# ppt0011/distributed_training

Hardware: AMD Instinct MI355X
Metric: images/sec (node) ResNet-50 at 1/2/4/8 MI355X; grad-sync bus GB/s (higher is better)
Workload: dtype bf16

## Files before the change

distributed_training_amd/_lib.py:

```python
from __future__ import annotations

import ctypes
import os
import threading

import torch

LIB_PATH = os.environ.get(
    "GSYNC_LIB", os.path.join(os.path.dirname(os.path.abspath(__file__)), "lib", "libgsync.so")
)

GS_OK = 0
GS_EINVAL, GS_EHIP, GS_ERCCL, GS_ESTATE, GS_ENOMEM, GS_ENODEV = -1, -2, -3, -4, -5, -6
GS_F32, GS_BF16, GS_F16, GS_F64, GS_I64, GS_I32, GS_U8 = 0, 1, 2, 3, 4, 5, 6
GS_DEV_HOST, GS_DEV_HIP = 0, 1
GS_SUM, GS_PROD, GS_MAX, GS_MIN, GS_AVG = 0, 1, 2, 3, 4
GS_SCALE_NONE, GS_SCALE_MUL, GS_SCALE_DIV = 0, 1, 2
GS_PLAN_SLOTS = 5
GS_RED_GROUPS = 64
GS_RED_PARTIALS = 1024
GS_BKT_AUTO_COLLECTIVE = 1
GS_BKT_GRAD_VIEW = 2
GS_BKT_NO_SCALE = 4
GS_BKT_REDUCE_SCATTER = 8
# ... 74 lines not shown
    "gs_rng_draw_u32": (_c_int, [_vp, _c_i64, _c_i64, _vp]),
    "gs_randperm": (_c_int, [ctypes.c_uint64, _c_i64, _vp]),
    "gs_distributed_sampler_indices": (_c_int, [_c_i64, _c_int, _c_int, _c_int, ctypes.c_uint64, _c_i64, _c_int,
                                                _vp, _c_i64, _p_i64]),
    "gs_crop_flip_params": (_c_int, [_vp, _c_i64, _c_int, _c_int, _c_int, _c_int, _c_int, _c_int, _vp, _c_i64,
                                     _vp]),
    "gs_image_augment": (_c_int, [_c_int, _c_int, _vp, _vp, _c_i64, _c_int, _c_int, _c_int, _c_int, _c_int, _c_int,
                                  _vp, _c_i64, _vp, _c_int, _c_int, _vp, _vp]),
    "gs_image_augment_mix": (_c_int, [_c_int, _c_int, _vp, _vp, _c_i64, _c_int, _c_int, _c_int, _c_int, _c_int, _c_int,
                                      _vp, _vp, _c_i64, _vp, _c_int, _c_int, _vp, _vp, _vp, _vp]),
    "gs_bn_bwd_partials": (_c_int, [_c_i64, _c_int]),
    "gs_bn_bwd_reduce": (_c_int, [_vp, _vp, _vp, _vp, _vp, _vp, _c_i64, _c_i64, _c_int, _vp]),
    "gs_bn_bwd_reduce_fork": (_c_int, [_vp, _vp, _vp, _vp, _vp, _vp, _vp, _c_i64, _c_i64, _c_int, _vp]),
    "gs_bn_bwd_dx": (_c_int, [_vp, _vp, _vp, _vp, _vp, _vp, _vp, _c_i64, _vp, _vp, _vp, _c_i64, _c_int, _vp]),
    "gs_add_relu_fwd": (_c_int, [_vp, _vp, _c_i64, _vp]),
    "gs_relu_maxpool_fwd": (_c_int, [_vp, _vp, _vp, _c_i64, _c_int, _c_int, _c_int, _vp]),
    "gs_maxpool_bwd": (_c_int, [_vp, _vp, _vp, _vp, _c_i64, _c_int, _c_int, _c_int, _vp]),
    "gs_relu_mask_fwd": (_c_int, [_vp, _vp, _c_i64, _vp]),
    "gs_add_relu_mask_fwd": (_c_int, [_vp, _vp, _vp, _c_i64, _vp]),
    "gs_relu_maxpool_mask_fwd": (_c_int, [_vp, _vp, _vp, _vp, _c_i64, _c_int, _c_int, _c_int, _vp]),
    "gs_bn_bwd_reduce_bits": (_c_int, [_vp, _vp, _vp, _vp, _vp, _vp, _c_i64, _c_i64, _c_int, _vp]),
    "gs_bn_bwd_reduce_fork_bits": (_c_int, [_vp, _vp, _vp, _vp, _vp, _vp, _vp, _c_i64, _c_i64, _c_int, _vp]),
    "gs_bn_bwd_dx_bits": (_c_int, [_vp, _vp, _vp, _vp, _vp, _vp, _vp, _c_i64, _vp, _vp, _vp, _c_i64, _c_int, _vp]),
    "gs_bn_infer_act": (_c_int, [_vp, _vp, _vp, _vp, _vp, _vp, _c_d, _c_int, _vp, _c_i64, _c_int, _vp]),
    "gs_bn_infer_relu_maxpool": (_c_int, [_vp, _vp, _vp, _vp, _vp, _c_d, _vp, _c_i64, _c_int, _c_int, _c_int, _vp]),
    "gs_eval_accumulate": (_c_int, [_c_int, _vp, _c_int, _vp, _c_i64, _c_i64, _c_i64, _c_i64, _p_i32, _c_int, _c_i64,
                                    _vp, _vp, _vp]),
    "gs_xent_fwd": (_c_int, [_c_int, _vp, _c_int, _vp, _c_i64, _c_i64, _c_i64, _c_i64, _c_f, _vp, _vp, _p_i32, _c_int,
                             _vp, _vp]),
    "gs_xent_bwd": (_c_int, [_c_int, _vp, _c_int, _vp, _c_i64, _c_i64, _c_i64, _c_i64, _c_f, _c_int, _vp, _vp, _vp, _vp,
                             _c_i64, _vp]),
    "gs_xent_mix_fwd": (_c_int, [_c_int, _vp, _c_int, _vp, _vp, _vp, _c_i64, _c_i64, _c_i64, _c_i64, _c_f, _vp, _vp,
                                 _p_i32, _c_int, _vp, _vp]),
    "gs_xent_mix_bwd": (_c_int, [_c_int, _vp, _c_int, _vp, _vp, _vp, _c_i64, _c_i64, _c_i64, _c_i64, _c_f, _c_int, _vp,
                                 _vp, _vp, _vp, _c_i64, _vp]),
    "gs_clip_coef":(_c_int, [_c_int, _vp, _c_f, _c_f, _vp, _vp, _vp]),
    "gs_unscale_check": (_c_int, [_vp, _c_int, _c_int, _vp, _vp, _vp]),
    "gs_sgd_step": (
        _c_int,
        [_vp, _c_int, _c_int, _c_d, _c_d, _c_d, _c_d, _c_int, _c_int, _c_int, _vp, _vp, _vp],
    ),
    "gs_adam_step": (
        _c_int,
        [_vp, _c_int, _c_int, _c_d, _c_d, _c_d, _c_d, _c_d, _c_int, _c_int, _c_d, _c_d, _vp, _vp, _vp],
    ),
    "gs_plan_set_adapt": (_c_int, [_vp, _p_i32]),
# ... 186 lines not shown
```

distributed_training_amd/csrc/gs_bn_kernels.hip:

```cpp
#include <hip/hip_runtime.h>

#include <algorithm>
#include <climits>
#include <cmath>

#include "gs_common.h"

#ifndef GS_BN_NT
#define GS_BN_NT 0
#endif
#ifndef GS_BN_DX_RNE
#define GS_BN_DX_RNE 0
#endif

namespace gs {
namespace {

#define HIP_RET(expr)                                                               \
  do {                                                                              \
    hipError_t _e = (expr);                                                         \
    if (_e != hipSuccess)                                                           \
      return fail(GS_EHIP, std::string(#expr " failed: ") + hipGetErrorString(_e)); \
  } while (0)

// ... 103 lines not shown
#pragma unroll
  for (int i = 0; i < 8; ++i) g[i] = yf[i] <= 0.f ? 0.f : g[i];
}

enum : int { kMaskNone = 0, kMaskY = 1, kMaskBits = 2 };

__device__ __forceinline__ void relu_mask_bits(float (&g)[8], uint32_t mb) {
#pragma unroll
  for (int i = 0; i < 8; ++i) g[i] = (mb >> i) & 1u ? g[i] : 0.f;
}

__device__ __forceinline__ uint8_t mask_byte(const float (&f)[8]) {
  uint32_t mb = 0;
#pragma unroll
  for (int j = 0; j < 8; ++j) mb |= (f[j] <= 0.f ? 0u : 1u) << j;
  return static_cast<uint8_t>(mb);
}

__device__ __forceinline__ void fork_sum(float (&g)[8], const bu4& bv) {
  float b[8];
  unpack8(bv, b);
#pragma unroll
  for (int i = 0; i < 8; ++i) g[i] = __uint_as_float(to_bf16(g[i] + b[i]) << 16);
}

template <int BLOCK, int MASK, bool WRITE_G, bool FORK>
__global__ void __launch_bounds__(BLOCK, (BLOCK == kBlock && MASK == kMaskBits && !WRITE_G) ? 5 : 1)
bn_bwd_reduce_kernel(const uint16_t* __restrict__ x, const uint16_t* __restrict__ dy, const uint16_t* __restrict__ dy2,
                     const uint16_t* __restrict__ y, const uint8_t* __restrict__ mask, uint16_t* __restrict__ gout,
                     const float* __restrict__ mean, float* __restrict__ ws, int64_t R, int C, int tx_log2,
                     int64_t rpb) {
  constexpr int U = FORK ? kBnForkUnroll : kBnUnroll;
  __shared__ float s_red[BLOCK * 16];
  __shared__ double s_grp[BLOCK];
  const int t = threadIdx.x;
  const int tx = 1 << tx_log2, ty = BLOCK >> tx_log2;
  const int tx_i = t & (tx - 1), ty_i = t >> tx_log2;
  const int v = blockIdx.x * tx + tx_i;
  const bool active = v < (C >> 3);
  const int c0 = v * 8;
  const int64_t r0 = static_cast<int64_t>(blockIdx.y) * rpb;
  const int64_t r1 = std::min<int64_t>(R, r0 + rpb);

  float sg[8], sq[8], m[8];
#pragma unroll
  for (int i = 0; i < 8; ++i) {
// ... 24 lines not shown
      uint32_t mb[U] = {};
#pragma unroll
      for (int k = 0; k < U; ++k) {
        xv[k] = ld16<false>(x + off + k * step);
        dv[k] = ld16<GS_BN_NT && WRITE_G>(dy + off + k * step);
        if constexpr (FORK) bv[k] = ld16<GS_BN_NT>(dy2 + off + k * step);
        if constexpr (MASK == kMaskY) yv[k] = ld16<GS_BN_NT && WRITE_G>(y + off + k * step);
        if constexpr (MASK == kMaskBits) mb[k] = mask[(off + k * step) >> 3];
      }
      if constexpr (MASK == kMaskBits) __builtin_amdgcn_sched_barrier(0);
#pragma unroll
      for (int k = 0; k < U; ++k) body(xv[k], dv[k], bv[k], yv[k], mb[k], off + k * step);
    }
    for (; r < r1; r += ty, off += step) {
      bu4 bv = {0u, 0u, 0u, 0u}, yv = {0u, 0u, 0u, 0u};
      uint32_t mb = 0;
      const bu4 xv = ld16<false>(x + off), dv = ld16<false>(dy + off);
      if constexpr (FORK) bv = ld16<false>(dy2 + off);
      if constexpr (MASK == kMaskY) yv = ld16<false>(y + off);
      if constexpr (MASK == kMaskBits) mb = mask[off >> 3];
      body(xv, dv, bv, yv, mb, off);
    }
  }
  const int F = 16 << tx_log2;
#pragma unroll
  for (int i = 0; i < 8; ++i) {
    s_red[t * 16 + 2 * i] = sg[i];
    s_red[t * 16 + 2 * i + 1] = sq[i];
  }
  __syncthreads();
  {
    const int o = t & (F - 1), grp = t >> (tx_log2 + 4);
    double a = 0.0;
#pragma unroll
    for (int k = 0; k < 16; ++k) a += static_cast<double>(s_red[(grp * 16 + k) * F + o]);
    s_grp[t] = a;
  }
  __syncthreads();
  if (t < F) {
    const int G = BLOCK / F;
    double a = 0.0;
    for (int k = 0; k < G; ++k) a += s_grp[k * F + t];
    const int ch = blockIdx.x * (tx * 8) + (t >> 1);
    if (ch < C) ws[(static_cast<int64_t>(blockIdx.y) * C + ch) * 2 + (t & 1)] = static_cast<float>(a);
  }
}

template <int BLOCK, int MASK>
__global__ void __launch_bounds__(BLOCK)
bn_bwd_dx_kernel(const uint16_t* __restrict__ x, const uint16_t* __restrict__ dy, const uint16_t* __restrict__ y,
                 const uint8_t* __restrict__ mask, const float* __restrict__ mean, const float* __restrict__ invstd, const float* __restrict__ weight,
                 const float* __restrict__ ws, int P, uint16_t* __restrict__ dx, float* __restrict__ gw,
                 float* __restrict__ gb, int64_t R, int C, int tx_log2, int64_t rpb, double inv_R) {
  __shared__ double s_fold[BLOCK * 4];
  __shared__ double s_sum[BLOCK / 2];
  const int t = threadIdx.x;
  const int tx = 1 << tx_log2, ty = BLOCK >> tx_log2;
  const int tx_i = t & (tx - 1), ty_i = t >> tx_log2;
  const int tile_c0 = blockIdx.x * (tx * 8);
  {
    const int F4 = 4 << tx_log2, G4 = BLOCK / F4;
    const int q = t & (F4 - 1), grp = t >> (tx_log2 + 2);
    double a[4] = {0.0, 0.0, 0.0, 0.0};
    if (tile_c0 + 2 * q < C) {
      const bf4* base = reinterpret_cast<const bf4*>(ws + static_cast<int64_t>(tile_c0) * 2) + q;
      const int64_t stride = C >> 1;
#pragma unroll 8
      for (int p = grp; p < P; p += G4) {
        const bf4 w4 = base[p * stride];
#pragma unroll
        for (int j = 0; j < 4; ++j) a[j] += static_cast<double>(w4[j]);
      }
    }
#pragma unroll
    for (int j = 0; j < 4; ++j) s_fold[t * 4 + j] = a[j];
    __syncthreads();
    if (t < 4 * F4) {
      double b = 0.0;
      for (int k = 0; k < G4; ++k) b += s_fold[k * 4 * F4 + t];
      s_sum[t] = b;
    }
    __syncthreads();
  }
  if (blockIdx.y == 0 && t < tx * 8 && tile_c0 + t < C) {
    gb[tile_c0 + t] = static_cast<float>(s_sum[2 * t]);
    gw[tile_c0 + t] = static_cast<float>(static_cast<double>(invstd[tile_c0 + t]) * s_sum[2 * t + 1]);
  }
  const int v = blockIdx.x * tx + tx_i;
  if (v >= (C >> 3)) return;
  const int c0 = v * 8;
  float m[8], a[8], m1[8], k2[8];
#pragma unroll
  for (int i = 0; i < 8; ++i) {
    const float is = invstd[c0 + i];
    m[i] = mean[c0 + i];
    a[i] = weight[c0 + i] * is;
    m1[i] = static_cast<float>(s_sum[tx_i * 16 + 2 * i] * inv_R);
    k2[i] = static_cast<float>(static_cast<double>(is) * is * s_sum[tx_i * 16 + 2 * i + 1] * inv_R);
  }
  auto body = [&](const bu4& xv, const bu4& dv, const bu4& yv, uint32_t mb, int64_t off) {
    float xf[8], g[8];
    unpack8(xv, xf);
    unpack8(dv, g);
    if constexpr (MASK == kMaskY) relu_mask(g, yv);
    if constexpr (MASK == kMaskBits) relu_mask_bits(g, mb);
#pragma unroll
// ... 7 lines not shown
  int64_t off = r * C + c0;
  for (; r + (kBnUnroll - 1) * ty < r1; r += kBnUnroll * ty, off += kBnUnroll * step) {
    bu4 xv[kBnUnroll], dv[kBnUnroll], yv[kBnUnroll] = {};
    uint32_t mb[kBnUnroll] = {};
#pragma unroll
    for (int k = 0; k < kBnUnroll; ++k) {
      xv[k] = ld16<GS_BN_NT>(x + off + k * step);
      dv[k] = ld16<GS_BN_NT>(dy + off + k * step);
      if constexpr (MASK == kMaskY) yv[k] = ld16<GS_BN_NT>(y + off + k * step);
      if constexpr (MASK == kMaskBits) mb[k] = mask[(off + k * step) >> 3];
    }
    if constexpr (MASK == kMaskBits) __builtin_amdgcn_sched_barrier(0);
#pragma unroll
    for (int k = 0; k < kBnUnroll; ++k) body(xv[k], dv[k], yv[k], mb[k], off + k * step);
  }
  for (; r < r1; r += ty, off += step) {
    bu4 yv = {0u, 0u, 0u, 0u};
    uint32_t mb = 0;
    const bu4 xv = ld16<false>(x + off), dv = ld16<false>(dy + off);
    if constexpr (MASK == kMaskY) yv = ld16<false>(y + off);
    if constexpr (MASK == kMaskBits) mb = mask[off >> 3];
    body(xv, dv, yv, mb, off);
  }
}

__device__ __forceinline__ float relu1(float v) { return v > 0.f ? v : (v != v ? v : 0.f); }

template <bool ADD, bool MASK>
__global__ void __launch_bounds__(kBlock)
add_relu_fwd_kernel(uint16_t* __restrict__ t, const uint16_t* __restrict__ id, uint8_t* __restrict__ mask,
                    int64_t nvec) {
  const int64_t base = static_cast<int64_t>(blockIdx.x) * (kBlock * kBnUnroll) + threadIdx.x;
  bu4 a[kBnUnroll], b[kBnUnroll] = {};
#pragma unroll
  for (int k = 0; k < kBnUnroll; ++k) {
    const int64_t i = base + k * kBlock;
    if (i < nvec) {
      a[k] = ld16<false>(t + i * 8);
      if constexpr (ADD) b[k] = ld16<false>(id + i * 8);
    }
  }
#pragma unroll
  for (int k = 0; k < kBnUnroll; ++k) {
    const int64_t i = base + k * kBlock;
    if (i < nvec) {
      float af[8];
// ... 525 lines not shown
    hipLaunchKernelGGL((relu_maxpool_fwd_kernel<false>), grid, block, 0, s, yp, pp, ip, mp, g.out_vecs, H, W, g.OH,
                       g.OW, C / 8);
  HIP_RET(hipGetLastError());
  return GS_OK;
}

}
}

extern "C" int gs_bn_bwd_dx(const void* x, const void* dy, const void* y, const float* mean, const float* invstd,
                            const float* weight, const float* ws, int64_t ws_floats, void* dx, float* grad_weight,
                            float* grad_bias, int64_t R, int C, void* stream) {
  return bn_dx("gs_bn_bwd_dx", x, dy, y, false, nullptr, mean, invstd, weight, ws, ws_floats, dx, grad_weight,
               grad_bias, R, C, stream);
}

extern "C" int gs_bn_bwd_dx_bits(const void* x, const void* dy, const void* mask, const float* mean,
                                 const float* invstd, const float* weight, const float* ws, int64_t ws_floats,
                                 void* dx, float* grad_weight, float* grad_bias, int64_t R, int C, void* stream) {
  return bn_dx("gs_bn_bwd_dx_bits", x, dy, nullptr, true, mask, mean, invstd, weight, ws, ws_floats, dx, grad_weight,
               grad_bias, R, C, stream);
}

extern "C" int gs_add_relu_fwd(void* t, const void* identity, int64_t n, void* stream) {
  return relu_tail("gs_add_relu_fwd", t, identity, true, nullptr, false, n, stream);
}

extern "C" int gs_add_relu_mask_fwd(void* t, const void* identity, void* mask, int64_t n, void* stream) {
  return relu_tail("gs_add_relu_mask_fwd", t, identity, true, mask, true, n, stream);
}

extern "C" int gs_relu_mask_fwd(void* t, void* mask, int64_t n, void* stream) {
  return relu_tail("gs_relu_mask_fwd", t, nullptr, false, mask, true, n, stream);
}

extern "C" int gs_relu_maxpool_fwd(const void* y, void* pooled, void* idx, int64_t N, int H, int W, int C,
                                   void* stream) {
  return relu_maxpool("gs_relu_maxpool_fwd", y, pooled, idx, nullptr, false, N, H, W, C, stream);
}

extern "C" int gs_relu_maxpool_mask_fwd(const void* y, void* pooled, void* idx, void* mask, int64_t N, int H, int W,
                                        int C, void* stream) {
  return relu_maxpool("gs_relu_maxpool_mask_fwd", y, pooled, idx, mask, true, N, H, W, C, stream);
}

extern "C" int gs_maxpool_bwd(const void* d_a, const void* d_b, const void* idx, void* dx, int64_t N, int H, int W,
// ... 80 lines not shown
```

distributed_training_amd/fused_bn.py:

```python
from __future__ import annotations

import contextlib
import os

import torch
import torch.nn.functional as F
from torch.autograd.function import once_differentiable

from . import _lib as L

last_path: str | None = None

_CL = torch.channels_last
_partials: dict = {}


def _n_partials(R: int, C: int) -> int:
    P = _partials.get((R, C))
    if P is None:
        P = _partials[(R, C)] = L.check(L.lib().gs_bn_bwd_partials(R, C), "gs_bn_bwd_partials")
    return P


def _mask_bits() -> bool:
# ... 126 lines not shown
        if dy_b is not None:
            g = torch.empty_like(x)
            fn = "gs_bn_bwd_reduce_fork_bits" if bits else "gs_bn_bwd_reduce_fork"
            L.check(getattr(lib, fn)(x.data_ptr(), dy.data_ptr(), dy_b.data_ptr(), yp, g.data_ptr(), mean.data_ptr(),
                                     ws.data_ptr(), ws.numel(), R, C, stream), fn)
            dy, yp = g, None
        elif ctx.has_residual:
            g = torch.empty_like(x)
            fn = "gs_bn_bwd_reduce_bits" if bits else "gs_bn_bwd_reduce"
            L.check(getattr(lib, fn)(x.data_ptr(), dy.data_ptr(), yp, g.data_ptr(), mean.data_ptr(), ws.data_ptr(),
                                     ws.numel(), R, C, stream), fn)
            dy, yp = g, None
        else:
            fn = "gs_bn_bwd_reduce_bits" if bits else "gs_bn_bwd_reduce"
            L.check(getattr(lib, fn)(x.data_ptr(), dy.data_ptr(), yp, None, mean.data_ptr(), ws.data_ptr(),
                                     ws.numel(), R, C, stream), fn)
        fn = "gs_bn_bwd_dx_bits" if bits and yp is not None else "gs_bn_bwd_dx"
        L.check(getattr(lib, fn)(x.data_ptr(), dy.data_ptr(), yp, mean.data_ptr(), invstd.data_ptr(),
                                 weight.data_ptr(), ws.data_ptr(), ws.numel(), dx.data_ptr(), gw.data_ptr(),
                                 gb.data_ptr(), R, C, stream), fn)
        return dx, gw, gb, g if ctx.has_residual else None, None, None, None, None


class _BnReluPool(torch.autograd.Function):

    @staticmethod
    def forward(ctx, x, weight, bias, bn, momentum, fork):
        y, mean, invstd, _, _ = torch._batch_norm_impl_index(
            x, weight, bias, bn.running_mean, bn.running_var, True, momentum, bn.eps, torch.backends.cudnn.enabled)
        if not y.is_contiguous(memory_format=_CL):
            raise RuntimeError("fused_bn: batch_norm returned a layout other than its channels_last input's")
        N, C, H, W = y.shape
        OH, OW = (H - 1) // 2 + 1, (W - 1) // 2 + 1
        out = torch.empty((N, C, OH, OW), dtype=y.dtype, device=y.device, memory_format=_CL)
        idx = torch.empty((N, OH, OW, C), dtype=torch.uint8, device=y.device)
        ctx.bits = _mask_bits()
        if ctx.bits:
            mask = torch.empty(y.numel() // 8, dtype=torch.uint8, device=y.device)
            L.check(L.lib().gs_relu_maxpool_mask_fwd(y.data_ptr(), out.data_ptr(), idx.data_ptr(), mask.data_ptr(), N,
                                                     H, W, C, L.stream_ptr(y.device)), "gs_relu_maxpool_mask_fwd")
            y = mask
        else:
            L.check(L.lib().gs_relu_maxpool_fwd(y.data_ptr(), out.data_ptr(), idx.data_ptr(), N, H, W, C,
                                                L.stream_ptr(y.device)), "gs_relu_maxpool_fwd")
        ctx.save_for_backward(x, weight, mean, invstd, y, idx)
        if fork:
# ... 45 lines not shown
def _pool_eligible(pool) -> bool:
    def is_(v, k):
        return v == k or v == (k, k) or v == [k, k]

    return (type(pool) is torch.nn.MaxPool2d and is_(pool.kernel_size, 3) and is_(pool.stride, 2)
            and is_(pool.padding, 1) and is_(pool.dilation, 1) and not pool.ceil_mode and not pool.return_indices
            and not (pool._forward_pre_hooks or pool._forward_hooks))


def bn_relu_pool(bn, x, pool, fork: bool = True):
    global last_path
    if _pool_eligible(pool) and _eval_eligible(bn, x, True, None):
        last_path = "fused_eval"
        out = _infer_relu_pool(bn, x)
        return (out, out) if fork else out
    if _pool_eligible(pool) and _eligible(bn, x, True, None):
        momentum = _bookkeeping(bn)
        last_path = "fused"
        return _BnReluPool.apply(x, bn.weight, bn.bias, bn, momentum, fork)
    out = pool(bn_act(bn, x))
    return (out, out) if fork else out


def bn_act(bn, x, relu: bool = True, residual=None, fork: bool = False):
    global last_path
    if _eval_eligible(bn, x, relu, residual):
        last_path = "fused_eval"
        out = _infer_act(bn, x, relu, residual)
        return (out, out) if fork else out
    if _eligible(bn, x, relu, residual):
        momentum = _bookkeeping(bn)
        last_path = "fused"
        return _BnAct.apply(x, bn.weight, bn.bias, residual, bn, momentum, relu, fork)
    last_path = "stock"
    out = bn(x)
    if residual is not None:
        out += residual
    if relu:
        out = F.relu(out, inplace=True)
    return (out, out) if fork else out
```

distributed_training_amd/resnet.py:

```python
from __future__ import annotations

import torch
import torch.nn as nn

from .fused_bn import bn_act, bn_relu_pool


def conv3x3(in_planes, out_planes, stride=1):
    return nn.Conv2d(in_planes, out_planes, kernel_size=3, stride=stride, padding=1, bias=False)


def conv1x1(in_planes, out_planes, stride=1):
    return nn.Conv2d(in_planes, out_planes, kernel_size=1, stride=stride, bias=False)


def _downsample(seq, x):
    return bn_act(seq[1], seq[0](x), relu=False)


class BasicBlock(nn.Module):
    expansion = 1

    def __init__(self, inplanes, planes, stride=1, downsample=None):
        super().__init__()
        self.conv1 = conv3x3(inplanes, planes, stride)
        self.bn1 = nn.BatchNorm2d(planes)
        self.relu = nn.ReLU(inplace=True)
        self.conv2 = conv3x3(planes, planes)
        self.bn2 = nn.BatchNorm2d(planes)
        self.downsample = downsample
        self.stride = stride

    def forward_pair(self, pair, fork_out):
        x, identity = pair
        if self.downsample is not None:
            identity = _downsample(self.downsample, identity)
        out = bn_act(self.bn1, self.conv1(x))
        return bn_act(self.bn2, self.conv2(out), residual=identity, fork=fork_out)

    def forward(self, x):
        return self.forward_pair((x, x), False)


class Bottleneck(nn.Module):
    expansion = 4

    def __init__(self, inplanes, planes, stride=1, downsample=None):
        super().__init__()
        self.conv1 = conv1x1(inplanes, planes)
        self.bn1 = nn.BatchNorm2d(planes)
        self.conv2 = conv3x3(planes, planes, stride)
        self.bn2 = nn.BatchNorm2d(planes)
        self.conv3 = conv1x1(planes, planes * self.expansion)
        self.bn3 = nn.BatchNorm2d(planes * self.expansion)
        self.relu = nn.ReLU(inplace=True)
        self.downsample = downsample
        self.stride = stride

    def forward_pair(self, pair, fork_out):
        x, identity = pair
        if self.downsample is not None:
            identity = _downsample(self.downsample, identity)
        out = bn_act(self.bn1, self.conv1(x))
        out = bn_act(self.bn2, self.conv2(out))
        return bn_act(self.bn3, self.conv3(out), residual=identity, fork=fork_out)

    def forward(self, x):
        return self.forward_pair((x, x), False)


class ResNet(nn.Module):
    def __init__(self, block, layers, num_classes=1000, width=64):
        super().__init__()
        self.inplanes = width
        self.conv1 = nn.Conv2d(3, self.inplanes, kernel_size=7, stride=2, padding=3, bias=False)
        self.bn1 = nn.BatchNorm2d(self.inplanes)
        self.relu = nn.ReLU(inplace=True)
        self.maxpool = nn.MaxPool2d(kernel_size=3, stride=2, padding=1)
        self.layer1 = self._make_layer(block, width, layers[0])
        self.layer2 = self._make_layer(block, width * 2, layers[1], stride=2)
        self.layer3 = self._make_layer(block, width * 4, layers[2], stride=2)
        self.layer4 = self._make_layer(block, width * 8, layers[3], stride=2)
        self.avgpool = nn.AdaptiveAvgPool2d((1, 1))
        self.fc = nn.Linear(width * 8 * block.expansion, num_classes)
        for m in self.modules():
            if isinstance(m, nn.Conv2d):
                nn.init.kaiming_normal_(m.weight, mode="fan_out", nonlinearity="relu")
            elif isinstance(m, (nn.BatchNorm2d, nn.GroupNorm)):
# ... 53 lines not shown
```

include/gsync.h:

```cpp
#ifndef GSYNC_H
#define GSYNC_H

#include <stdint.h>

#ifdef __cplusplus
extern "C" {
#endif

#define GSYNC_VERSION 1000

#define GS_OK 0
#define GS_EINVAL (-1)
#define GS_EHIP (-2)
#define GS_ERCCL (-3)
#define GS_ESTATE (-4)
#define GS_ENOMEM (-5)
#define GS_ENODEV (-6)

#define GS_F32 0
#define GS_BF16 1
#define GS_F16 2
#define GS_F64 3
#define GS_I64 4
#define GS_I32 5
// ... 200 lines not shown
int gs_bn_bwd_partials(int64_t R, int C);
int gs_bn_bwd_reduce(const void* x, const void* dy, const void* y, void* g_out, const float* mean, float* ws,
                     int64_t ws_floats, int64_t R, int C, void* stream);
int gs_bn_bwd_reduce_fork(const void* x, const void* dy_a, const void* dy_b, const void* y, void* g_out,
                          const float* mean, float* ws, int64_t ws_floats, int64_t R, int C, void* stream);
int gs_bn_bwd_dx(const void* x, const void* dy, const void* y, const float* mean, const float* invstd,
                 const float* weight, const float* ws, int64_t ws_floats, void* dx, float* grad_weight,
                 float* grad_bias, int64_t R, int C, void* stream);
int gs_add_relu_fwd(void* t, const void* identity, int64_t n, void* stream);
int gs_relu_maxpool_fwd(const void* y, void* pooled, void* idx, int64_t N, int H, int W, int C, void* stream);
int gs_maxpool_bwd(const void* d_a, const void* d_b, const void* idx, void* dx, int64_t N, int H, int W, int C,
                   void* stream);
int gs_relu_mask_fwd(void* t, void* mask, int64_t n, void* stream);
int gs_add_relu_mask_fwd(void* t, const void* identity, void* mask, int64_t n, void* stream);
int gs_relu_maxpool_mask_fwd(const void* y, void* pooled, void* idx, void* mask, int64_t N, int H, int W, int C,
                             void* stream);
int gs_bn_bwd_reduce_bits(const void* x, const void* dy, const void* mask, void* g_out, const float* mean, float* ws,
                          int64_t ws_floats, int64_t R, int C, void* stream);
int gs_bn_bwd_reduce_fork_bits(const void* x, const void* dy_a, const void* dy_b, const void* mask, void* g_out,
                               const float* mean, float* ws, int64_t ws_floats, int64_t R, int C, void* stream);
int gs_bn_bwd_dx_bits(const void* x, const void* dy, const void* mask, const float* mean, const float* invstd,
                      const float* weight, const float* ws, int64_t ws_floats, void* dx, float* grad_weight,
                      float* grad_bias, int64_t R, int C, void* stream);

int gs_bn_infer_act(const void* x, const void* residual, const float* running_mean, const float* running_var,
                    const float* weight, const float* bias, double eps, int relu, void* y, int64_t R, int C,
                    void* stream);
int gs_bn_infer_relu_maxpool(const void* x, const float* running_mean, const float* running_var, const float* weight,
                             const float* bias, double eps, void* pooled, int64_t N, int H, int W, int C,
                             void* stream);
int gs_eval_accumulate(int device_kind, const void* logits, int logits_dtype, const int64_t* labels, int64_t B,
                       int64_t K, int64_t row_stride, int64_t n_valid, const int32_t* topk, int n_topk,
                       int64_t ignore_index, void* ws, void* acc, void* stream);

int gs_xent_fwd(int device_kind, const void* logits, int logits_dtype, const int64_t* labels, int64_t B, int64_t K,
                int64_t row_stride, int64_t ignore_index, float label_smoothing, void* rows, void* red,
                const int32_t* topk, int n_topk, void* acc, void* stream);
int gs_xent_bwd(int device_kind, const void* logits, int logits_dtype, const int64_t* labels, int64_t B, int64_t K,
                int64_t row_stride, int64_t ignore_index, float label_smoothing, int reduction, const void* rows,
                const void* red, const float* grad_out, void* dlogits, int64_t d_row_stride, void* stream);
int gs_xent_mix_fwd(int device_kind, const void* logits, int logits_dtype, const int64_t* labels_a,
                    const int64_t* labels_b, const float* lam, int64_t B, int64_t K, int64_t row_stride,
                    int64_t ignore_index, float label_smoothing, void* rows, void* red, const int32_t* topk,
                    int n_topk, void* acc, void* stream);
int gs_xent_mix_bwd(int device_kind, const void* logits, int logits_dtype, const int64_t* labels_a,
                    const int64_t* labels_b, const float* lam, int64_t B, int64_t K, int64_t row_stride,
// ... 8 lines not shown
```

Measured before the change: 7262.

## Fuse main and downsample BatchNorm backward in residual blocks into paired kernels

New measurement: 7332 (median of 6 runs). No clear change (+1.0%).

```diff
diff --git a/distributed_training_amd/_lib.py b/distributed_training_amd/_lib.py
--- a/distributed_training_amd/_lib.py
+++ b/distributed_training_amd/_lib.py
@@ -120,6 +120,9 @@
     "gs_bn_bwd_reduce_bits": (_c_int, [_vp, _vp, _vp, _vp, _vp, _vp, _c_i64, _c_i64, _c_int, _vp]),
     "gs_bn_bwd_reduce_fork_bits": (_c_int, [_vp, _vp, _vp, _vp, _vp, _vp, _vp, _c_i64, _c_i64, _c_int, _vp]),
     "gs_bn_bwd_dx_bits": (_c_int, [_vp, _vp, _vp, _vp, _vp, _vp, _vp, _c_i64, _vp, _vp, _vp, _c_i64, _c_int, _vp]),
+    "gs_bn_bwd_reduce_pair_bits": (_c_int, [_vp, _vp, _vp, _vp, _vp, _vp, _vp, _vp, _vp, _vp, _c_i64, _c_i64, _c_int,
+                                            _vp]),
+    "gs_bn_bwd_dx_pair": (_c_int, [_vp] * 11 + [_c_i64] + [_vp] * 6 + [_c_i64, _c_int, _vp]),
     "gs_bn_infer_act": (_c_int, [_vp, _vp, _vp, _vp, _vp, _vp, _c_d, _c_int, _vp, _c_i64, _c_int, _vp]),
     "gs_bn_infer_relu_maxpool": (_c_int, [_vp, _vp, _vp, _vp, _vp, _c_d, _vp, _c_i64, _c_int, _c_int, _c_int, _vp]),
     "gs_eval_accumulate": (_c_int, [_c_int, _vp, _c_int, _vp, _c_i64, _c_i64, _c_i64, _c_i64, _p_i32, _c_int, _c_i64,
diff --git a/distributed_training_amd/csrc/gs_bn_kernels.hip b/distributed_training_amd/csrc/gs_bn_kernels.hip
--- a/distributed_training_amd/csrc/gs_bn_kernels.hip
+++ b/distributed_training_amd/csrc/gs_bn_kernels.hip
@@ -149,6 +149,35 @@
   unpack8(bv, b);
 #pragma unroll
   for (int i = 0; i < 8; ++i) g[i] = __uint_as_float(to_bf16(g[i] + b[i]) << 16);
+}
+
+template <int BLOCK>
+__device__ __forceinline__ void reduce_fold(float* s_red, double* s_grp, const float (&sg)[8], const float (&sq)[8],
+                                            float* __restrict__ ws, int C, int tx_log2) {
+  const int t = threadIdx.x;
+  const int tx = 1 << tx_log2;
+  const int F = 16 << tx_log2;
+#pragma unroll
+  for (int i = 0; i < 8; ++i) {
+    s_red[t * 16 + 2 * i] = sg[i];
+    s_red[t * 16 + 2 * i + 1] = sq[i];
+  }
+  __syncthreads();
+  {
+    const int o = t & (F - 1), grp = t >> (tx_log2 + 4);
+    double a = 0.0;
+#pragma unroll
+    for (int k = 0; k < 16; ++k) a += static_cast<double>(s_red[(grp * 16 + k) * F + o]);
+    s_grp[t] = a;
+  }
+  __syncthreads();
+  if (t < F) {
+    const int G = BLOCK / F;
+    double a = 0.0;
+    for (int k = 0; k < G; ++k) a += s_grp[k * F + t];
+    const int ch = blockIdx.x * (tx * 8) + (t >> 1);
+    if (ch < C) ws[(static_cast<int64_t>(blockIdx.y) * C + ch) * 2 + (t & 1)] = static_cast<float>(a);
+  }
 }
 
 template <int BLOCK, int MASK, bool WRITE_G, bool FORK>
@@ -219,28 +248,35 @@
       body(xv, dv, bv, yv, mb, off);
     }
   }
-  const int F = 16 << tx_log2;
-#pragma unroll
-  for (int i = 0; i < 8; ++i) {
-    s_red[t * 16 + 2 * i] = sg[i];
-    s_red[t * 16 + 2 * i + 1] = sq[i];
-  }
+  reduce_fold<BLOCK>(s_red, s_grp, sg, sq, ws, C, tx_log2);
+}
+
+template <int BLOCK>
+__device__ __forceinline__ void dx_fold(const float* __restrict__ ws, int P, int C, int tile_c0, int tx_log2,
+                                        double* s_fold, double* s_sum) {
+  const int t = threadIdx.x;
+  const int F4 = 4 << tx_log2, G4 = BLOCK / F4;
+  const int q = t & (F4 - 1), grp = t >> (tx_log2 + 2);
+  double a[4] = {0.0, 0.0, 0.0, 0.0};
+  if (tile_c0 + 2 * q < C) {
+    const bf4* base = reinterpret_cast<const bf4*>(ws + static_cast<int64_t>(tile_c0) * 2) + q;
+    const int64_t stride = C >> 1;
+#pragma unroll 8
+    for (int p = grp; p < P; p += G4) {
+      const bf4 w4 = base[p * stride];
+#pragma unroll
+      for (int j = 0; j < 4; ++j) a[j] += static_cast<double>(w4[j]);
+    }
+  }
+#pragma unroll
+  for (int j = 0; j < 4; ++j) s_fold[t * 4 + j] = a[j];
   __syncthreads();
-  {
-    const int o = t & (F - 1), grp = t >> (tx_log2 + 4);
-    double a = 0.0;
-#pragma unroll
-    for (int k = 0; k < 16; ++k) a += static_cast<double>(s_red[(grp * 16 + k) * F + o]);
-    s_grp[t] = a;
+  if (t < 4 * F4) {
+    double b = 0.0;
+    for (int k = 0; k < G4; ++k) b += s_fold[k * 4 * F4 + t];
+    s_sum[t] = b;
   }
   __syncthreads();
-  if (t < F) {
-    const int G = BLOCK / F;
-    double a = 0.0;
-    for (int k = 0; k < G; ++k) a += s_grp[k * F + t];
-    const int ch = blockIdx.x * (tx * 8) + (t >> 1);
-    if (ch < C) ws[(static_cast<int64_t>(blockIdx.y) * C + ch) * 2 + (t & 1)] = static_cast<float>(a);
-  }
 }
 
 template <int BLOCK, int MASK>
@@ -255,30 +291,7 @@
   const int tx = 1 << tx_log2, ty = BLOCK >> tx_log2;
   const int tx_i = t & (tx - 1), ty_i = t >> tx_log2;
   const int tile_c0 = blockIdx.x * (tx * 8);
-  {
-    const int F4 = 4 << tx_log2, G4 = BLOCK / F4;
-    const int q = t & (F4 - 1), grp = t >> (tx_log2 + 2);
-    double a[4] = {0.0, 0.0, 0.0, 0.0};
-    if (tile_c0 + 2 * q < C) {
-      const bf4* base = reinterpret_cast<const bf4*>(ws + static_cast<int64_t>(tile_c0) * 2) + q;
-      const int64_t stride = C >> 1;
-#pragma unroll 8
-      for (int p = grp; p < P; p += G4) {
-        const bf4 w4 = base[p * stride];
-#pragma unroll
-        for (int j = 0; j < 4; ++j) a[j] += static_cast<double>(w4[j]);
-      }
-    }
-#pragma unroll
-    for (int j = 0; j < 4; ++j) s_fold[t * 4 + j] = a[j];
-    __syncthreads();
-    if (t < 4 * F4) {
-      double b = 0.0;
-      for (int k = 0; k < G4; ++k) b += s_fold[k * 4 * F4 + t];
-      s_sum[t] = b;
-    }
-    __syncthreads();
-  }
+  dx_fold<BLOCK>(ws, P, C, tile_c0, tx_log2, s_fold, s_sum);
   if (blockIdx.y == 0 && t < tx * 8 && tile_c0 + t < C) {
     gb[tile_c0 + t] = static_cast<float>(s_sum[2 * t]);
     gw[tile_c0 + t] = static_cast<float>(static_cast<double>(invstd[tile_c0 + t]) * s_sum[2 * t + 1]);
@@ -332,6 +345,155 @@
     if constexpr (MASK == kMaskBits) mb = mask[off >> 3];
     body(xv, dv, yv, mb, off);
   }
+}
+
+#ifndef GS_BN_PAIR_UNROLL
+#define GS_BN_PAIR_UNROLL 2
+#endif
+constexpr int kBnPairUnroll = GS_BN_PAIR_UNROLL;
+
+template <int BLOCK, bool FORK>
+__global__ void __launch_bounds__(BLOCK)
+bn_bwd_reduce_pair_kernel(const uint16_t* __restrict__ xa, const uint16_t* __restrict__ xb,
+                          const uint16_t* __restrict__ dy, const uint16_t* __restrict__ dy2,
+                          const uint8_t* __restrict__ mask, uint16_t* __restrict__ gout,
+                          const float* __restrict__ mean_a, const float* __restrict__ mean_b, float* __restrict__ ws_a,
+                          float* __restrict__ ws_b, int64_t R, int C, int tx_log2, int64_t rpb) {
+  constexpr int U = kBnPairUnroll;
+  __shared__ float s_red[BLOCK * 16];
+  __shared__ double s_grp[BLOCK];
+  const int t = threadIdx.x;
+  const int tx = 1 << tx_log2, ty = BLOCK >> tx_log2;
+  const int tx_i = t & (tx - 1), ty_i = t >> tx_log2;
+  const int v = blockIdx.x * tx + tx_i;
+  const bool active = v < (C >> 3);
+  const int c0 = v * 8;
+  const int64_t r0 = static_cast<int64_t>(blockIdx.y) * rpb;
+  const int64_t r1 = std::min<int64_t>(R, r0 + rpb);
+
+  float sg[8], sqa[8], sqb[8], ma[8], mb[8];
+#pragma unroll
+  for (int i = 0; i < 8; ++i) {
+    sg[i] = sqa[i] = sqb[i] = 0.f;
+    ma[i] = active ? mean_a[c0 + i] : 0.f;
+    mb[i] = active ? mean_b[c0 + i] : 0.f;
+  }
+  auto body = [&](const bu4& xav, const bu4& xbv, const bu4& dv, const bu4& bv, uint32_t bits, int64_t off) {
+    float xf[8], g[8];
+    unpack8(dv, g);
+    if constexpr (FORK) fork_sum(g, bv);
+    relu_mask_bits(g, bits);
+    st16(gout + off, pack8_exact(g));
+    unpack8(xav, xf);
+#pragma unroll
+    for (int i = 0; i < 8; ++i) {
+      sg[i] += g[i];
+      sqa[i] = fmaf(g[i], xf[i] - ma[i], sqa[i]);
+    }
+    unpack8(xbv, xf);
+#pragma unroll
+    for (int i = 0; i < 8; ++i) sqb[i] = fmaf(g[i], xf[i] - mb[i], sqb[i]);
+  };
+  if (active) {
+    const int64_t step = static_cast<int64_t>(ty) * C;
+    int64_t r = r0 + ty_i;
+    int64_t off = r * C + c0;
+    for (; r + (U - 1) * ty < r1; r += U * ty, off += U * step) {
+      bu4 xav[U], xbv[U], dv[U], bv[U] = {};
+      uint32_t bits[U];
+#pragma unroll
+      for (int k = 0; k < U; ++k) {
+        xav[k] = ld16<false>(xa + off + k * step);
+        xbv[k] = ld16<false>(xb + off + k * step);
+        dv[k] = ld16<GS_BN_NT>(dy + off + k * step);
+        if constexpr (FORK) bv[k] = ld16<GS_BN_NT>(dy2 + off + k * step);
+        bits[k] = mask[(off + k * step) >> 3];
+      }
+#pragma unroll
+      for (int k = 0; k < U; ++k) body(xav[k], xbv[k], dv[k], bv[k], bits[k], off + k * step);
+    }
+    for (; r < r1; r += ty, off += step) {
+      bu4 bv = {0u, 0u, 0u, 0u};
+      const bu4 xav = ld16<false>(xa + off), xbv = ld16<false>(xb + off), dv = ld16<false>(dy + off);
+      if constexpr (FORK) bv = ld16<false>(dy2 + off);
+      body(xav, xbv, dv, bv, mask[off >> 3], off);
+    }
+  }
+  reduce_fold<BLOCK>(s_red, s_grp, sg, sqa, ws_a, C, tx_log2);
+  reduce_fold<BLOCK>(s_red, s_grp, sg, sqb, ws_b, C, tx_log2);
+}
+
+template <int BLOCK>
+__global__ void __launch_bounds__(BLOCK)
+bn_bwd_dx_pair_kernel(const uint16_t* __restrict__ xa, const uint16_t* __restrict__ xb, const uint16_t* __restrict__ g,
+                      const float* __restrict__ mean_a, const float* __restrict__ invstd_a,
+                      const float* __restrict__ weight_a, const float* __restrict__ mean_b,
+                      const float* __restrict__ invstd_b, const float* __restrict__ weight_b,
+                      const float* __restrict__ ws_a, const float* __restrict__ ws_b, int P, uint16_t* __restrict__ dxa,
+                      uint16_t* __restrict__ dxb, float* __restrict__ gw_a, float* __restrict__ gb_a,
+                      float* __restrict__ gw_b, float* __restrict__ gb_b, int64_t R, int C, int tx_log2, int64_t rpb,
+                      double inv_R) {
+  constexpr int U = kBnPairUnroll;
+  __shared__ double s_fold[BLOCK * 4];
+  __shared__ double s_sum_a[BLOCK / 2];
+  __shared__ double s_sum_b[BLOCK / 2];
+  const int t = threadIdx.x;
+  const int tx = 1 << tx_log2, ty = BLOCK >> tx_log2;
+  const int tx_i = t & (tx - 1), ty_i = t >> tx_log2;
+  const int tile_c0 = blockIdx.x * (tx * 8);
+  dx_fold<BLOCK>(ws_a, P, C, tile_c0, tx_log2, s_fold, s_sum_a);
+  dx_fold<BLOCK>(ws_b, P, C, tile_c0, tx_log2, s_fold, s_sum_b);
+  if (blockIdx.y == 0 && t < tx * 8 && tile_c0 + t < C) {
+    gb_a[tile_c0 + t] = static_cast<float>(s_sum_a[2 * t]);
+    gw_a[tile_c0 + t] = static_cast<float>(static_cast<double>(invstd_a[tile_c0 + t]) * s_sum_a[2 * t + 1]);
+    gb_b[tile_c0 + t] = static_cast<float>(s_sum_b[2 * t]);
+    gw_b[tile_c0 + t] = static_cast<float>(static_cast<double>(invstd_b[tile_c0 + t]) * s_sum_b[2 * t + 1]);
+  }
+  const int v = blockIdx.x * tx + tx_i;
+  if (v >= (C >> 3)) return;
+  const int c0 = v * 8;
+  float ma[8], aa[8], m1a[8], k2a[8], mb[8], ab[8], m1b[8], k2b[8];
+#pragma unroll
+  for (int i = 0; i < 8; ++i) {
+    const float isa = invstd_a[c0 + i], isb = invstd_b[c0 + i];
+    ma[i] = mean_a[c0 + i];
+    aa[i] = weight_a[c0 + i] * isa;
+    m1a[i] = static_cast<float>(s_sum_a[tx_i * 16 + 2 * i] * inv_R);
+    k2a[i] = static_cast<float>(static_cast<double>(isa) * isa * s_sum_a[tx_i * 16 + 2 * i + 1] * inv_R);
+    mb[i] = mean_b[c0 + i];
+    ab[i] = weight_b[c0 + i] * isb;
+    m1b[i] = static_cast<float>(s_sum_b[tx_i * 16 + 2 * i] * inv_R);
+    k2b[i] = static_cast<float>(static_cast<double>(isb) * isb * s_sum_b[tx_i * 16 + 2 * i + 1] * inv_R);
+  }
+  auto body = [&](const bu4& xav, const bu4& xbv, const bu4& gv, int64_t off) {
+    float xf[8], gf[8], o[8];
+    unpack8(gv, gf);
+    unpack8(xav, xf);
+#pragma unroll
+    for (int i = 0; i < 8; ++i) o[i] = aa[i] * fmaf(ma[i] - xf[i], k2a[i], gf[i] - m1a[i]);
+    st16(dxa + off, pack8_dx(o));
+    unpack8(xbv, xf);
+#pragma unroll
+    for (int i = 0; i < 8; ++i) o[i] = ab[i] * fmaf(mb[i] - xf[i], k2b[i], gf[i] - m1b[i]);
+    st16(dxb + off, pack8_dx(o));
+  };
+  const int64_t r0 = static_cast<int64_t>(blockIdx.y) * rpb;
+  const int64_t r1 = std::min<int64_t>(R, r0 + rpb);
+  const int64_t step = static_cast<int64_t>(ty) * C;
+  int64_t r = r0 + ty_i;
+  int64_t off = r * C + c0;
+  for (; r + (U - 1) * ty < r1; r += U * ty, off += U * step) {
+    bu4 xav[U], xbv[U], gv[U];
+#pragma unroll
+    for (int k = 0; k < U; ++k) {
+      xav[k] = ld16<GS_BN_NT>(xa + off + k * step);
+      xbv[k] = ld16<GS_BN_NT>(xb + off + k * step);
+      gv[k] = ld16<GS_BN_NT>(g + off + k * step);
+    }
+#pragma unroll
+    for (int k = 0; k < U; ++k) body(xav[k], xbv[k], gv[k], off + k * step);
+  }
+  for (; r < r1; r += ty, off += step) body(ld16<false>(xa + off), ld16<false>(xb + off), ld16<false>(g + off), off);
 }
 
 __device__ __forceinline__ float relu1(float v) { return v > 0.f ? v : (v != v ? v : 0.f); }
@@ -903,6 +1065,102 @@
                grad_bias, R, C, stream);
 }
 
+#define GS_BN_PAIR_LAUNCH(LAUNCH)          \
+  do {                                     \
+    if constexpr (kBnTileVecs >= 32) {     \
+      if (geom.block == 4 * kBlock) {      \
+        LAUNCH(4 * kBlock);                \
+        break;                             \
+      }                                    \
+    }                                      \
+    if constexpr (kBnTileVecs >= 16) {     \
+      if (geom.block == 2 * kBlock) {      \
+        LAUNCH(2 * kBlock);                \
+        break;                             \
+      }                                    \
+    }                                      \
+    LAUNCH(kBlock);                        \
+  } while (0)
+
+extern "C" int gs_bn_bwd_reduce_pair_bits(const void* x_a, const void* x_b, const void* dy, const void* dy2,
+                                          const void* mask, void* g_out, const float* mean_a, const float* mean_b,
+                                          float* ws_a, float* ws_b, int64_t ws_floats, int64_t R, int C,
+                                          void* stream) {
+  const std::string w("gs_bn_bwd_reduce_pair_bits");
+  GS_TRY_RET(check_shape(R, C));
+  GS_CHECK_ARG(x_a && x_b && dy && mask && g_out && mean_a && mean_b && ws_a && ws_b, w + ": null pointer");
+  GS_CHECK_ARG(aligned16(x_a) && aligned16(x_b) && aligned16(dy) && aligned16(dy2) && aligned16(g_out) &&
+                   aligned16(ws_a) && aligned16(ws_b),
+               w + ": pointers must be 16-byte aligned");
+  const int64_t bytes = R * C * 2;
+  GS_CHECK_ARG(!overlap(g_out, x_a, bytes) && !overlap(g_out, x_b, bytes) && !overlap(g_out, dy, bytes) &&
+                   !overlap(g_out, dy2, bytes),
+               w + ": g_out overlaps an input");
+  GS_CHECK_ARG(!overlap(g_out, bytes, mask, R * C / 8), w + ": g_out overlaps the mask");
+  const BnGeom geom = bn_geom(R, C);
+  const int64_t need = static_cast<int64_t>(geom.P) * C * 2;
+  GS_CHECK_ARG(ws_floats >= need, w + ": workspace too small");
+  GS_CHECK_ARG(!overlap(ws_a, need * 4, ws_b, need * 4), w + ": the workspaces overlap");
+  const dim3 grid(geom.ctiles, geom.P), block(geom.block);
+  hipStream_t s = static_cast<hipStream_t>(stream);
+  const uint16_t* ap = static_cast<const uint16_t*>(x_a);
+  const uint16_t* bp = static_cast<const uint16_t*>(x_b);
+  const uint16_t* dp = static_cast<const uint16_t*>(dy);
+  const uint16_t* d2 = static_cast<const uint16_t*>(dy2);
+  const uint8_t* mp = static_cast<const uint8_t*>(mask);
+  uint16_t* gp = static_cast<uint16_t*>(g_out);
+#define GS_BN_PAIR_REDUCE_FORK(BLOCK)                                                                              \
+  hipLaunchKernelGGL((bn_bwd_reduce_pair_kernel<BLOCK, true>), grid, block, 0, s, ap, bp, dp, d2, mp, gp, mean_a, \
+                     mean_b, ws_a, ws_b, R, C, geom.tx_log2, geom.rpb)
+#define GS_BN_PAIR_REDUCE(BLOCK)                                                                                    \
+  hipLaunchKernelGGL((bn_bwd_reduce_pair_kernel<BLOCK, false>), grid, block, 0, s, ap, bp, dp, d2, mp, gp, mean_a, \
+                     mean_b, ws_a, ws_b, R, C, geom.tx_log2, geom.rpb)
+  if (d2) GS_BN_PAIR_LAUNCH(GS_BN_PAIR_REDUCE_FORK);
+  else GS_BN_PAIR_LAUNCH(GS_BN_PAIR_REDUCE);
+#undef GS_BN_PAIR_REDUCE
+#undef GS_BN_PAIR_REDUCE_FORK
+  HIP_RET(hipGetLastError());
+  return GS_OK;
+}
+
+extern "C" int gs_bn_bwd_dx_pair(const void* x_a, const void* x_b, const void* g, const float* mean_a,
+                                 const float* invstd_a, const float* weight_a, const float* mean_b,
+                                 const float* invstd_b, const float* weight_b, const float* ws_a, const float* ws_b,
+                                 int64_t ws_floats, void* dx_a, void* dx_b, float* gw_a, float* gb_a, float* gw_b,
+                                 float* gb_b, int64_t R, int C, void* stream) {
+  const std::string w("gs_bn_bwd_dx_pair");
+  GS_TRY_RET(check_shape(R, C));
+  GS_CHECK_ARG(x_a && x_b && g && mean_a && invstd_a && weight_a && mean_b && invstd_b && weight_b && ws_a && ws_b &&
+                   dx_a && dx_b && gw_a && gb_a && gw_b && gb_b,
+               w + ": null pointer");
+  GS_CHECK_ARG(aligned16(x_a) && aligned16(x_b) && aligned16(g) && aligned16(dx_a) && aligned16(dx_b) &&
+                   aligned16(ws_a) && aligned16(ws_b),
+               w + ": pointers must be 16-byte aligned");
+  const int64_t bytes = R * C * 2;
+  GS_CHECK_ARG(!overlap(dx_a, dx_b, bytes), w + ": dx_a overlaps dx_b");
+  for (const void* in : {x_a, x_b, g})
+    GS_CHECK_ARG(!overlap(dx_a, in, bytes) && !overlap(dx_b, in, bytes), w + ": dx overlaps an input");
+  const BnGeom geom = bn_geom(R, C);
+  GS_CHECK_ARG(ws_floats >= static_cast<int64_t>(geom.P) * C * 2, w + ": workspace too small");
+  const dim3 grid(geom.ctiles, geom.P), block(geom.block);
+  hipStream_t s = static_cast<hipStream_t>(stream);
+  const uint16_t* ap = static_cast<const uint16_t*>(x_a);
+  const uint16_t* bp = static_cast<const uint16_t*>(x_b);
+  const uint16_t* gp = static_cast<const uint16_t*>(g);
+  uint16_t* oa = static_cast<uint16_t*>(dx_a);
+  uint16_t* ob = static_cast<uint16_t*>(dx_b);
+  const double inv_R = 1.0 / static_cast<double>(R);
+#define GS_BN_PAIR_DX(BLOCK)                                                                                        \
+  hipLaunchKernelGGL((bn_bwd_dx_pair_kernel<BLOCK>), grid, block, 0, s, ap, bp, gp, mean_a, invstd_a, weight_a,    \
+                     mean_b, invstd_b, weight_b, ws_a, ws_b, geom.P, oa, ob, gw_a, gb_a, gw_b, gb_b, R, C,         \
+                     geom.tx_log2, geom.rpb, inv_R)
+  GS_BN_PAIR_LAUNCH(GS_BN_PAIR_DX);
+#undef GS_BN_PAIR_DX
+  HIP_RET(hipGetLastError());
+  return GS_OK;
+}
+#undef GS_BN_PAIR_LAUNCH
+
 extern "C" int gs_add_relu_fwd(void* t, const void* identity, int64_t n, void* stream) {
   return relu_tail("gs_add_relu_fwd", t, identity, true, nullptr, false, n, stream);
 }
diff --git a/distributed_training_amd/fused_bn.py b/distributed_training_amd/fused_bn.py
--- a/distributed_training_amd/fused_bn.py
+++ b/distributed_training_amd/fused_bn.py
@@ -172,6 +172,59 @@
         return dx, gw, gb, g if ctx.has_residual else None, None, None, None, None
 
 
+class _BnActPair(torch.autograd.Function):
+
+    @staticmethod
+    def forward(ctx, x, weight, bias, x_ds, weight_ds, bias_ds, bn, bn_ds, momentum, momentum_ds, fork):
+        enabled = torch.backends.cudnn.enabled
+        res, mean_ds, invstd_ds, _, _ = torch._batch_norm_impl_index(
+            x_ds, weight_ds, bias_ds, bn_ds.running_mean, bn_ds.running_var, True, momentum_ds, bn_ds.eps, enabled)
+        y, mean, invstd, _, _ = torch._batch_norm_impl_index(
+            x, weight, bias, bn.running_mean, bn.running_var, True, momentum, bn.eps, enabled)
+        if not (y.is_contiguous(memory_format=_CL) and res.is_contiguous(memory_format=_CL)):
+            raise RuntimeError("fused_bn: batch_norm returned a layout other than its channels_last input's")
+        mask = torch.empty(y.numel() // 8, dtype=torch.uint8, device=y.device)
+        L.check(L.lib().gs_add_relu_mask_fwd(y.data_ptr(), res.data_ptr(), mask.data_ptr(), y.numel(),
+                                             L.stream_ptr(y.device)), "gs_add_relu_mask_fwd")
+        ctx.save_for_backward(x, weight, mean, invstd, x_ds, weight_ds, mean_ds, invstd_ds, mask)
+        if fork:
+            ctx.set_materialize_grads(False)
+            return y, y.view_as(y)
+        return y
+
+    @staticmethod
+    @once_differentiable
+    def backward(ctx, dy, dy_b=None):
+        x, weight, mean, invstd, x_ds, weight_ds, mean_ds, invstd_ds, mask = ctx.saved_tensors
+        if dy is None:
+            dy, dy_b = dy_b, None
+        if dy is None:
+            return (None,) * 11
+        if not dy.is_contiguous(memory_format=_CL):
+            dy = dy.contiguous(memory_format=_CL)
+        if dy_b is not None and not dy_b.is_contiguous(memory_format=_CL):
+            dy_b = dy_b.contiguous(memory_format=_CL)
+        C = x.shape[1]
+        R = x.numel() // C
+        n = _n_partials(R, C) * C * 2
+        ws = torch.empty(2 * n, dtype=torch.float32, device=x.device)
+        ws_a, ws_b = ws[:n], ws[n:]
+        g = torch.empty_like(x)
+        dx, dx_ds = torch.empty_like(x), torch.empty_like(x_ds)
+        gw, gb, gw_ds, gb_ds = (torch.empty_like(weight) for _ in range(4))
+        lib, stream = L.lib(), L.stream_ptr(x.device)
+        L.check(lib.gs_bn_bwd_reduce_pair_bits(x.data_ptr(), x_ds.data_ptr(), dy.data_ptr(),
+                                               None if dy_b is None else dy_b.data_ptr(), mask.data_ptr(),
+                                               g.data_ptr(), mean.data_ptr(), mean_ds.data_ptr(), ws_a.data_ptr(),
+                                               ws_b.data_ptr(), n, R, C, stream), "gs_bn_bwd_reduce_pair_bits")
+        L.check(lib.gs_bn_bwd_dx_pair(x.data_ptr(), x_ds.data_ptr(), g.data_ptr(), mean.data_ptr(), invstd.data_ptr(),
+                                      weight.data_ptr(), mean_ds.data_ptr(), invstd_ds.data_ptr(),
+                                      weight_ds.data_ptr(), ws_a.data_ptr(), ws_b.data_ptr(), n, dx.data_ptr(),
+                                      dx_ds.data_ptr(), gw.data_ptr(), gb.data_ptr(), gw_ds.data_ptr(),
+                                      gb_ds.data_ptr(), R, C, stream), "gs_bn_bwd_dx_pair")
+        return dx, gw, gb, dx_ds, gw_ds, gb_ds, None, None, None, None, None
+
+
 class _BnReluPool(torch.autograd.Function):
 
     @staticmethod
@@ -263,6 +316,25 @@
     return (out, out) if fork else out
 
 
+pair_enabled = True
+
+
+def pair_eligible(bn, x, bn_ds, x_ds) -> bool:
+    return (pair_enabled and _mask_bits() and x.shape == x_ds.shape and x.device == x_ds.device
+            and _eligible(bn_ds, x_ds, False, None) and _eligible(bn, x, True, None))
+
+
+def bn_act_pair(bn, x, bn_ds, x_ds, fork: bool = False):
+    global last_path
+    if pair_eligible(bn, x, bn_ds, x_ds):
+        momentum_ds = _bookkeeping(bn_ds)
+        momentum = _bookkeeping(bn)
+        last_path = "fused"
+        return _BnActPair.apply(x, bn.weight, bn.bias, x_ds, bn_ds.weight, bn_ds.bias, bn, bn_ds, momentum,
+                                momentum_ds, fork)
+    return bn_act(bn, x, residual=bn_act(bn_ds, x_ds, relu=False), fork=fork)
+
+
 def bn_act(bn, x, relu: bool = True, residual=None, fork: bool = False):
     global last_path
     if _eval_eligible(bn, x, relu, residual):
diff --git a/distributed_training_amd/resnet.py b/distributed_training_amd/resnet.py
--- a/distributed_training_amd/resnet.py
+++ b/distributed_training_amd/resnet.py
@@ -3,7 +3,7 @@
 import torch
 import torch.nn as nn
 
-from .fused_bn import bn_act, bn_relu_pool
+from .fused_bn import bn_act, bn_act_pair, bn_relu_pool, pair_eligible
 
 
 def conv3x3(in_planes, out_planes, stride=1):
@@ -16,6 +16,27 @@
 
 def _downsample(seq, x):
     return bn_act(seq[1], seq[0](x), relu=False)
+
+
+def _is_conv_bn(seq):
+    return (type(seq) is nn.Sequential and len(seq) == 2 and isinstance(seq[0], nn.Conv2d)
+            and isinstance(seq[1], nn.BatchNorm2d))
+
+
+def _branch(seq, identity):
+    if seq is None:
+        return identity, None
+    if _is_conv_bn(seq):
+        return None, seq[0](identity)
+    return _downsample(seq, identity), None
+
+
+def _tail(seq, bn, out, identity, x_ds, fork_out):
+    if x_ds is not None:
+        if pair_eligible(bn, out, seq[1], x_ds):
+            return bn_act_pair(bn, out, seq[1], x_ds, fork=fork_out)
+        identity = bn_act(seq[1], x_ds, relu=False)
+    return bn_act(bn, out, residual=identity, fork=fork_out)
 
 
 class BasicBlock(nn.Module):
@@ -33,10 +54,9 @@
 
     def forward_pair(self, pair, fork_out):
         x, identity = pair
-        if self.downsample is not None:
-            identity = _downsample(self.downsample, identity)
+        identity, x_ds = _branch(self.downsample, identity)
         out = bn_act(self.bn1, self.conv1(x))
-        return bn_act(self.bn2, self.conv2(out), residual=identity, fork=fork_out)
+        return _tail(self.downsample, self.bn2, self.conv2(out), identity, x_ds, fork_out)
 
     def forward(self, x):
         return self.forward_pair((x, x), False)
@@ -59,11 +79,10 @@
 
     def forward_pair(self, pair, fork_out):
         x, identity = pair
-        if self.downsample is not None:
-            identity = _downsample(self.downsample, identity)
+        identity, x_ds = _branch(self.downsample, identity)
         out = bn_act(self.bn1, self.conv1(x))
         out = bn_act(self.bn2, self.conv2(out))
-        return bn_act(self.bn3, self.conv3(out), residual=identity, fork=fork_out)
+        return _tail(self.downsample, self.bn3, self.conv3(out), identity, x_ds, fork_out)
 
     def forward(self, x):
         return self.forward_pair((x, x), False)
diff --git a/include/gsync.h b/include/gsync.h
--- a/include/gsync.h
+++ b/include/gsync.h
@@ -246,6 +246,14 @@
 int gs_bn_bwd_dx_bits(const void* x, const void* dy, const void* mask, const float* mean, const float* invstd,
                       const float* weight, const float* ws, int64_t ws_floats, void* dx, float* grad_weight,
                       float* grad_bias, int64_t R, int C, void* stream);
+int gs_bn_bwd_reduce_pair_bits(const void* x_a, const void* x_b, const void* dy, const void* dy2, const void* mask,
+                               void* g_out, const float* mean_a, const float* mean_b, float* ws_a, float* ws_b,
+                               int64_t ws_floats, int64_t R, int C, void* stream);
+int gs_bn_bwd_dx_pair(const void* x_a, const void* x_b, const void* g, const float* mean_a, const float* invstd_a,
+                      const float* weight_a, const float* mean_b, const float* invstd_b, const float* weight_b,
+                      const float* ws_a, const float* ws_b, int64_t ws_floats, void* dx_a, void* dx_b,
+                      float* grad_weight_a, float* grad_bias_a, float* grad_weight_b, float* grad_bias_b, int64_t R,
+                      int C, void* stream);
 
 int gs_bn_infer_act(const void* x, const void* residual, const float* running_mean, const float* running_var,
                     const float* weight, const float* bias, double eps, int relu, void* y, int64_t R, int C,
```
